# gyhandy/Neural-Sim-NeRF

Measured on AMD Instinct MI355X. Metric: Mray-samples/sec at 400x400, 64+128 samples, 8x256 MLP, higher is better.
Workload: dtype f16x2

## Files before the change

### neural_sim_nerf_amd/csrc/nsr_kernels.hip

```cpp
#include <hip/hip_runtime.h>
#include <stdint.h>
#include "nsr_device.h"

#if !defined(NSR_UNIT_F32) && !defined(NSR_UNIT_H2) && !defined(NSR_UNIT_B3) && !defined(NSR_UNIT_X16)
#define NSR_UNIT_F32 1
#define NSR_UNIT_H2 1
#define NSR_UNIT_B3 1
#define NSR_UNIT_X16 1
#endif
#ifndef NSR_UNIT_F32
#define NSR_UNIT_F32 0
#endif
#ifndef NSR_UNIT_H2
#define NSR_UNIT_H2 0
#endif
#ifndef NSR_UNIT_B3
#define NSR_UNIT_B3 0
#endif
#ifndef NSR_UNIT_X16
#define NSR_UNIT_X16 0
#endif
#define NSR_CAT_(a, b) a##b
#define NSR_CAT(a, b) NSR_CAT_(a, b)

// ... 88 lines not shown
#pragma unroll
  for (int c = 0; c < 4; ++c) A0[c] = *(const f32x4*)(p + c * 1024);
}

template <int U>
__device__ __forceinline__ void ring_load_quarter(const Ring& rg, f32x4 (&A)[4], int lane) {
  const char* p = rg.smem + rg.cslot * kSlabBytes + U * kStepBytes + lane * 16;
#pragma unroll
  for (int c = 0; c < 4; ++c) A[c] = *(const f32x4*)(p + c * 1024);
}

template <int NS = kRingSlots>
__device__ __forceinline__ void ring_advance(Ring& rg, f32x4 (&A)[4], int lane) {
  asm volatile("s_waitcnt vmcnt(%0) lgkmcnt(0)" ::"n"(4 * (NS - 2)) : "memory");
#ifndef NSR_EXP_NOBARRIER
  __builtin_amdgcn_s_barrier();
#endif
  rg.cslot = (rg.cslot + 1 == NS) ? 0 : rg.cslot + 1;
  const char* p = rg.smem + rg.cslot * kSlabBytes + lane * 16;
#pragma unroll
  for (int c = 0; c < 4; ++c) A[c] = *(const f32x4*)(p + c * 1024);
}

#define NSR_MFMA(a, b, c) __builtin_amdgcn_mfma_f32_32x32x2f32((a), (b), (c), 0, 0, 0)
__device__ __forceinline__ f32x16 mfma_op(float a, float b, f32x16 c) { return __builtin_amdgcn_mfma_f32_32x32x2f32(a, b, c, 0, 0, 0); }
__device__ __forceinline__ f32x4 mfma_op(float a, float b, f32x4 c) { return __builtin_amdgcn_mfma_f32_16x16x4f32(a, b, c, 0, 0, 0); }

template <int NMO, int KK0, int KK1, bool ZERO = false, int NACC, typename BOp, typename AccT>
__device__ __forceinline__ void consume(const f32x4 (&A)[4], int step, BOp bop, AccT (&acc)[NACC]) {
#pragma unroll
  for (int kk = KK0; kk < KK1; ++kk)
#pragma unroll
    for (int c = 0; c < 4; ++c) {
      const int n = 4 * step + c, tq = n / NMO, mo = n % NMO;
      if (ZERO && tq == 0 && kk == 0) acc[mo] = mfma_op(A[c][kk], bop(4 * tq + kk), AccT{0});
      else acc[mo] = mfma_op(A[c][kk], bop(4 * tq + kk), acc[mo]);
    }
}

#define NSR_PIN() __builtin_amdgcn_sched_barrier(0)
#define NSR_SGB(mask, n) __builtin_amdgcn_sched_group_barrier((mask), (n), 0)
#define NSR_MASK_VALU 0x002
#define NSR_MASK_SALU 0x004
#define NSR_MASK_MFMA 0x008
#define NSR_MASK_VMEM 0x010
#define NSR_MASK_DSRD 0x100
template <int N_MFMA>
__device__ __forceinline__ void step_pattern() {
#pragma unroll
  for (int i = 0; i < N_MFMA; ++i) {
    NSR_SGB(NSR_MASK_MFMA, 1);
    NSR_SGB(NSR_MASK_DSRD, 1);
    NSR_SGB(NSR_MASK_VALU, 2);
  }
}
template <int N_MFMA>
__device__ __forceinline__ void step_pattern_dma() {
#pragma unroll
  for (int i = 0; i < N_MFMA; ++i) {
    NSR_SGB(NSR_MASK_MFMA, 1);
    NSR_SGB(NSR_MASK_DSRD, 1);
    NSR_SGB(NSR_MASK_VMEM, 1);
    NSR_SGB(NSR_MASK_SALU, 3);
    NSR_SGB(NSR_MASK_VALU, 2);
  }
}

template <int NMO, int NTQ, int NS = kRingSlots, bool ZERO = false, int NACC, typename BOp, typename AccT>
__device__ __forceinline__ void seg(Ring& rg, f32x4 (&A0)[4], f32x4 (&A1)[4], BOp bop, AccT (&acc)[NACC],
                                    int lane) {
  static_assert((NMO * NTQ) % 16 == 0, "a segment is a whole number of slabs");
#pragma unroll
  for (int s = 0; s < NMO * NTQ / 4; s += 4) {
    NSR_PIN(); ring_load_quarter<1>(rg, A1, lane); consume<NMO, 0, 4, ZERO>(A0, s, bop, acc);     step_pattern<16>();
    NSR_PIN(); ring_load_quarter<2>(rg, A0, lane); consume<NMO, 0, 4, ZERO>(A1, s + 1, bop, acc); step_pattern<16>();
    NSR_PIN(); ring_load_quarter<3>(rg, A1, lane); consume<NMO, 0, 4, ZERO>(A0, s + 2, bop, acc); step_pattern<16>();
    NSR_PIN(); consume<NMO, 0, 1, ZERO>(A1, s + 3, bop, acc);
    NSR_PIN(); ring_advance<NS>(rg, A0, lane);
    ring_issue<NS>(rg); consume<NMO, 1, 4, ZERO>(A1, s + 3, bop, acc); step_pattern_dma<12>();
    NSR_PIN();
  }
}

template <int NG>
struct BRegs16 {
  const f32x16 (&v)[NG];
  __device__ __forceinline__ float operator()(int t) const { return v[t >> 4][t & 15]; }
};
template <int N>
struct BArr {
  const float (&v)[N];
  __device__ __forceinline__ float operator()(int t) const { return v[t]; }
};
struct BViews {
  const f32x16 (&v)[8];
  const float (&ed)[16];
  __device__ __forceinline__ float operator()(int t) const { return t < 128 ? v[(t & 127) >> 4][t & 15] : ed[t & 15]; }
};

__device__ __forceinline__ int aux_half(int lane) { return opaque_v((lane >> 5) * 4); }

template <int NMO>
__device__ __forceinline__ void load_bias(const float* bias, int h4 , f32x16 (&acc)[NMO]) {
#pragma unroll
  for (int mo = 0; mo < NMO; ++mo)
#pragma unroll
    for (int rq = 0; rq < 4; ++rq) {
      f32x4 v = *(const f32x4*)(bias + (mo * 4 + rq) * 8 + h4);
      acc[mo][rq * 4 + 0] = v[0];
      acc[mo][rq * 4 + 1] = v[1];
      acc[mo][rq * 4 + 2] = v[2];
      acc[mo][rq * 4 + 3] = v[3];
    }
}

#include "nsr_b3.inc"
#include "nsr_h2.inc"

constexpr int kMlpF32 = 0;
constexpr int kMlpB3 = 1;
constexpr int kMlpH2 = 2;

template <int NMO>
__device__ __forceinline__ uint4 relu_mask(const f32x16 (&acc)[NMO]) {
  unsigned w[4] = {0u, 0u, 0u, 0u};
#pragma unroll
  for (int mo = 0; mo < NMO; ++mo)
#pragma unroll
    for (int r = 0; r < 16; ++r) {
      const int on = max(__float_as_int(acc[mo][r]), 0) - 1;
      w[mo >> 1] = __builtin_amdgcn_alignbit(w[mo >> 1], (unsigned)on, 31);
    }
  return make_uint4(w[0], w[1], w[2], w[3]);
}

__device__ __forceinline__ float enc_trig(float a, int k) {
  const double kMagic = 6755399441055744.0;
  const double t = (double)a * 0.63661977236758134308;
  const double tm = t + kMagic;
  const int n = __double2loint(tm) + k;
  const double f = t - (tm - kMagic);
  const float r = (float)(f * 1.57079632679489661923);
  const float z = r * r;
  float ps = __builtin_fmaf(-1.9515295891e-4f, z, 8.3321608736e-3f);
  ps = __builtin_fmaf(ps, z, -1.6666654611e-1f);
  ps = __builtin_fmaf(ps * z, r, r);
  float pc = __builtin_fmaf(2.443315711809948e-5f, z, -1.388731625493765e-3f);
  pc = __builtin_fmaf(pc, z, 4.166664568298827e-2f);
  pc = __builtin_fmaf(pc * z, z, __builtin_fmaf(-0.5f, z, 1.0f));
  const float v = (n & 1) ? pc : ps;
  return __uint_as_float(__float_as_uint(v) ^ ((unsigned)(n & 2) << 30));
}

__device__ __forceinline__ float enc_domain(float x, int nfreq) {
  return __builtin_fabsf(x) < ldexpf(1.0f, 25 - nfreq) ? x : __builtin_nanf("");
}

__device__ __forceinline__ float enc_poison(float px, float py, float pz, float vx, float vy, float vz) {
  const float a = (enc_domain(px, kMultires) * 0.0f + enc_domain(py, kMultires) * 0.0f) + enc_domain(pz, kMultires) * 0.0f;
  const float b = (enc_domain(vx, kMultiresViews) * 0.0f + enc_domain(vy, kMultiresViews) * 0.0f) +
                  enc_domain(vz, kMultiresViews) * 0.0f;
  return __builtin_fabsf(a + b);
}

template <bool CAPTURE, int MODE = kMlpF32>
__device__ __forceinline__ void mlp_pass(Ring& rg, const float* aux, f32x4 (&A0)[4], f32x4 (&A1)[4], int lane,
                                         float px, float py, float pz, float vx, float vy, float vz,
                                         float (&raw)[4], uint4* mask_dst = nullptr , int mask_tid = 0,
                                         long long* tp = nullptr ) {
#ifdef NSR_PHASE_TIMING
  long long tpl = clock64();
#define NSR_TP(i) do { if (tp) { const long long t_ = clock64(); tp[i] += t_ - tpl; tpl = t_; } } while (0)
#else
#define NSR_TP(i) do { } while (0)
#endif
  const int h = lane >> 5;
  const int h4 = aux_half(lane);
  const float poison = enc_poison(px, py, pz, vx, vy, vz);
  float e[32];
  float ed[16];
  {
    const float p[3] = {px, py, pz};
    const float v[3] = {vx, vy, vz};
#pragma unroll
    for (int L = 0; L < kMultires; ++L)
#pragma unroll
      for (int ax = 0; ax < 3; ++ax) e[3 * L + ax] = enc_trig(enc_domain(p[ax], kMultires) * (float)(1 << L), h);
#pragma unroll
    for (int L = 0; L < kMultiresViews; ++L)
#pragma unroll
      for (int ax = 0; ax < 3; ++ax) ed[3 * L + ax] = enc_trig(enc_domain(v[ax], kMultiresViews) * (float)(1 << L), h);
    e[30] = h ? pz : px;
    e[31] = h ? 0.0f : py;
    ed[12] = h ? vz : vx;
    ed[13] = h ? 0.0f : vy;
    ed[14] = 0.0f;
    ed[15] = 0.0f;
  }

  f32x16 acc[8];
  f32x16 in[8];
  auto enc_src = [&](int kb, int i) { return e[(8 * kb + i) & 31]; };
  auto in_src = [&](int kb, int i) { return in[(kb >> 1) & 7][8 * (kb & 1) + i]; };
  constexpr bool B3 = MODE == kMlpB3;
  constexpr bool H2M = MODE == kMlpH2;
  float amax = 0.0f;
  const float* h2s = aux + kAuxH2Scale;
#if NSR_H2_SCHED == 3 && !defined(NSR_EXP_H2_NOFRAG) && !defined(NSR_EXP_H2_HALFBARRIER) && !defined(NSR_EXP_H2_NOSPLIT)
  constexpr bool TAIL = H2M && !CAPTURE;
#else
  constexpr bool TAIL = false;
#endif
  static_assert(kAuxBiasV == kAuxBias + 9 * 256, "the views layer's bias follows feature_linear's: 'bias of layer L + 1' for L = 8");
  NSR_TP(0);
  load_bias<8>(aux + kAuxBias, h4, acc);
  NSR_TP(2);
  if constexpr (B3) gemm_b3<8, 2>(rg, A0, A1, enc_src, acc, lane);
  else if constexpr (TAIL)
    gemm_h2_tail<4>(rg, A0, A1, enc_src, H2Scale{{h2s[0], 0.0f}, 4}, acc, lane, amax, H2Tail{acc, in, 0, h2_lds_base(aux + kAuxBias + 256, h4)});
  else if constexpr (H2M) gemm_h2<8, 4>(rg, A0, A1, enc_src, H2Scale{{h2s[0], 0.0f}, 4}, acc, lane, amax);
  else seg<8, 8>(rg, A0, A1, BArr<32>{e}, acc, lane);
  NSR_TP(1);
  if (CAPTURE) mask_dst[mask_tid] = relu_mask<8>(acc);
  if constexpr (!TAIL) {
#pragma unroll
    for (int mo = 0; mo < 8; ++mo) in[mo] = relu16(acc[mo]);
  }

  float alpha_part = 0.0f;
#pragma unroll 1
  for (int L = 1; L <= 8; ++L) {
    if constexpr (!TAIL) load_bias<8>(aux + kAuxBias + L * 256, h4, acc);
    NSR_TP(2);
    if (L == 5) {
      if constexpr (B3) gemm_b3<8, 2>(rg, A0, A1, enc_src, acc, lane);
      else if constexpr (H2M) gemm_h2<8, 4>(rg, A0, A1, enc_src, H2Scale{{h2s[9], 0.0f}, 4}, acc, lane, amax);
      else seg<8, 8>(rg, A0, A1, BArr<32>{e}, acc, lane);
      NSR_TP(1);
    }
    if (L == 8) {
      const float* wa = aux + kAuxWAlpha;
#pragma unroll
      for (int tq = 0; tq < 32; ++tq) {
        f32x4 w = *(const f32x4*)(wa + tq * 8 + h4);
#pragma unroll
        for (int kk = 0; kk < 4; ++kk)
          alpha_part = __builtin_fmaf(w[kk], in[(4 * tq + kk) >> 4][(4 * tq + kk) & 15], alpha_part);
      }
    }
    if constexpr (B3) gemm_b3<8, 8>(rg, A0, A1, in_src, acc, lane);
    else if constexpr (TAIL)
      gemm_h2_tail<16>(rg, A0, A1, in_src, H2Scale{{h2s[L], 0.0f}, 16}, acc, lane, amax,
                       H2Tail{acc, in, (L == 8) ? (int)0x80000000 : 0, h2_lds_base(aux + kAuxBias + (L + 1) * 256, h4)});
    else if constexpr (H2M) gemm_h2<8, 16>(rg, A0, A1, in_src, H2Scale{{h2s[L], 0.0f}, 16}, acc, lane, amax);
    else seg<8, 32>(rg, A0, A1, BRegs16<8>{in}, acc, lane);
    NSR_TP(1);
    if (CAPTURE && L < 8) mask_dst[L * 256 + mask_tid] = relu_mask<8>(acc);
    if constexpr (!TAIL) {
      const int thr = (L == 8) ? (int)0x80000000 : 0;
#pragma unroll
      for (int mo = 0; mo < 8; ++mo) in[mo] = clamp_bits16(acc[mo], thr);
    }
  }

  f32x16 av[4];
  if constexpr (TAIL) {
#pragma unroll
    for (int mo = 0; mo < 4; ++mo) av[mo] = acc[mo];
  } else {
    load_bias<4>(aux + kAuxBiasV, h4, av);
  }
  NSR_TP(2);
  if constexpr (B3) {
    auto v_src = [&](int kb, int i) {
      return kb < 16 ? in[(kb >> 1) & 7][8 * (kb & 1) + i] : (kb < 18 ? ed[(8 * (kb - 16) + i) & 15] : 0.0f);
    };
    gemm_b3<4, 5>(rg, A0, A1, v_src, av, lane);
  } else if constexpr (H2M) {
    auto v_src = [&](int kb, int i) { return kb < 16 ? in[(kb >> 1) & 7][8 * (kb & 1) + i] : ed[(8 * (kb - 16) + i) & 15]; };
    gemm_h2<4, 18>(rg, A0, A1, v_src, H2Scale{{h2s[10], h2s[11]}, 16}, av, lane, amax);
  } else {
    seg<4, 36>(rg, A0, A1, BViews{in, ed}, av, lane);
  }
  NSR_TP(1);
  if (CAPTURE) mask_dst[8 * 256 + mask_tid] = relu_mask<4>(av);

  float part[4] = {0.0f, 0.0f, 0.0f, alpha_part};
  if constexpr (H2M) {
    const float ov = amax > kH2Max ? __builtin_nanf("") : 0.0f;
    part[0] = part[1] = part[2] = ov;
    part[3] = alpha_part + ov;
  }
#pragma unroll
  for (int c = 0; c < 3; ++c) {
    const float* wr = aux + kAuxWRgb + c * 128;
#pragma unroll
    for (int mo = 0; mo < 4; ++mo)
#pragma unroll
      for (int rq = 0; rq < 4; ++rq) {
        f32x4 w = *(const f32x4*)(wr + (mo * 4 + rq) * 8 + h4);
#pragma unroll
        for (int ri = 0; ri < 4; ++ri)
          part[c] = __builtin_fmaf(w[ri], fmaxf(av[mo][rq * 4 + ri], 0.0f), part[c]);
      }
  }
#pragma unroll
  for (int c = 0; c < 4; ++c) {
    float other = __shfl_xor(part[c], 32);
    float lo_half = h ? other : part[c];
    float hi_half = h ? part[c] : other;
    raw[c] = ((lo_half + hi_half) + aux[(c < 3) ? (kAuxBRgb + c) : kAuxBAlpha]) + poison;
  }
  NSR_TP(3);
#undef NSR_TP
}

template <int NSS, int NFS>
struct ItemStateT {
  static constexpr int kNS = NSS, kNF = NFS;
  float tcoarse[NSS];
  float ufine[128];
  float ray[2][16];
  float zc[2][NSS];
  float rawc[2][NSS][4];
  float w0[2][NSS];
  float cdf[2][NSS];
  float zs[2][128];
  float zf[2][NFS];
  float rawf[2][NFS][4];
  float alpha[2][NFS];
  float wf[2][NFS];
  float tf[2][NFS];
  float om[2][NFS];
  float bwd_scratch[2][NFS][2];
  float psum[2][NFS / 32][12];
  float gnorm[2];
  float res[2][8];
};
typedef ItemStateT<64, 192> ItemState;
typedef ItemStateT<128, 256> ItemStateBig;
static_assert(sizeof(ItemState) == 23048, "the YCB-V layout is part of the shipped kernels' LDS budget");
template <int NS> struct ItemStateFor { typedef ItemState type; };
template <> struct ItemStateFor<128> { typedef ItemStateBig type; };

__device__ __forceinline__ float sigmoidf_(float x) { return 1.0f / (1.0f + expf(-x)); }

template <int S, int R = 2, int STRIDE = S, typename ST>
__device__ __forceinline__ void composite(ST& st, const float* z, float* raw, float* wout, float* tout, int tid,
                                          const float* noise = nullptr ,
                                          long long row0 = 0, int valid = R) {
  static_assert(S % 8 == 0, "scan is unrolled by 8");
  for (int idx = tid; idx < R * S; idx += 256) {
    const int r = idx / S, i = idx - r * S;
    const float* zr = z + r * STRIDE;
    float dist = (i < S - 1) ? (zr[i + 1] - zr[i]) : 1e10f;
    dist = dist * st.ray[r][11];
    float* q = raw + (r * STRIDE + i) * 4;
    if (noise) q[3] = q[3] + noise[(row0 + (r < valid ? r : 0)) * S + i];
    const float sigma = fmaxf(q[3], 0.0f);
    const float a = 1.0f - expf(-sigma * dist);
    st.alpha[r][i] = a;
    st.om[r][i] = (1.0f - a) + 1e-10f;
    q[0] = sigmoidf_(q[0]);
    q[1] = sigmoidf_(q[1]);
    q[2] = sigmoidf_(q[2]);
  }
  __syncthreads();
  if ((tid & 63) == 0 && tid < 64 * R) {
    const int r = tid >> 6;
    double T = 1.0;
#pragma unroll 1
    for (int i0 = 0; i0 < S; i0 += 8) {
      double f[8];
#pragma unroll
      for (int k = 0; k < 8; ++k) f[k] = (double)st.om[r][i0 + k];
#pragma unroll
      for (int k = 0; k < 8; ++k) {
        tout[r * STRIDE + i0 + k] = (float)T;
        T = T * f[k];
      }
    }
  }
  __syncthreads();
  if (tid < 64 * R) {
    const int r = tid >> 6, l = tid & 63;
    const float* zr = z + r * STRIDE;
    const float* q = raw + r * STRIDE * 4;
    float cr = 0.f, cg = 0.f, cb = 0.f, depth = 0.f, acc = 0.f;
#pragma unroll
    for (int i = l; i < S; i += 64) {
      const float w = st.alpha[r][i] * tout[r * STRIDE + i];
      wout[r * STRIDE + i] = w;
      cr = cr + w * q[i * 4 + 0];
      cg = cg + w * q[i * 4 + 1];
      cb = cb + w * q[i * 4 + 2];
      depth = depth + w * zr[i];
      acc = acc + w;
    }
#pragma unroll
    for (int m = 32; m >= 1; m >>= 1) {
      cr += __shfl_xor(cr, m); cg += __shfl_xor(cg, m); cb += __shfl_xor(cb, m);
      depth += __shfl_xor(depth, m); acc += __shfl_xor(acc, m);
    }
    if (l == 0) {
      const float qd = depth / acc;
      float disp;
      if (qd != qd) disp = qd;
      else disp = 1.0f / fmaxf(1e-10f, qd);
      if (st.ray[r][12] != 0.0f) {
        const float bg = 1.0f - acc;
        cr = cr + bg; cg = cg + bg; cb = cb + bg;
      }
      st.res[r][0] = cr; st.res[r][1] = cg; st.res[r][2] = cb;
      st.res[r][3] = disp; st.res[r][4] = acc; st.res[r][5] = depth;
    }
  }
  __syncthreads();
}
// ... 253 lines not shown
      const float upper = i < NS - 1 ? 0.5f * (zr[i + 1] + zr[i]) : zr[NS - 1];
      zn = lower + (upper - lower) * t_rand[(row0 + (r < valid ? r : 0)) * NS + i];
    }
    __syncthreads();
    if (tid < 2 * NS) st.zc[r][i] = zn;
    __syncthreads();
  }
}

__device__ __forceinline__ void gen_ray(const float* __restrict__ c2w, float fx, float fy, float cx, float cy,
                                        int row, int col, float (&o)[3], float (&d)[3]) {
  const float dx = ((float)col - cx) / fx;
  const float dy = -(((float)row - cy) / fy);
  const float dz = -1.0f;
#pragma unroll
  for (int a = 0; a < 3; ++a) {
    d[a] = ((dx * c2w[a * 4 + 0]) + (dy * c2w[a * 4 + 1])) + (dz * c2w[a * 4 + 2]);
    o[a] = c2w[a * 4 + 3];
  }
}

struct RenderArgs {
  const float* nets;
  long long net_stride;
  const float* aux[2];
  const float* tcoarse;
  const float* ufine;
  const float* rays_o;
  const float* rays_d;
  const float* c2w;
  float fx, fy, cx, cy;
  int H, W;
  long long n_rays;
  float near_, far_;
  int fine;
  int camera;
  int white_bkgd;
  int lindisp;
  float *rgb, *disp, *acc, *rgb0, *disp0, *acc0, *z_std;
  float *dbg_w0, *dbg_zs, *dbg_zf, *dbg_raw0, *dbg_raw;
  long long* dbg_inds;
  float* zf_scratch;
  int chunk;
  unsigned* sched_flags;
  unsigned* status;
  int super_lg;
  int spin_max;
  unsigned epoch;
  unsigned* epoch_counter;
  unsigned long long* work_counter;
  const float* viewdirs;
  const float* t_rand;
  const float* u_rays;
  const float* noise0;
  const float* noise1;
  const float* near_rays;
  const float* far_rays;
  unsigned long long* ovf_items;
  unsigned* ovf_stat;
  unsigned ovf_cap;
  const unsigned long long* item_list;
  const unsigned* item_count;
  unsigned item_cap;
};

__device__ __forceinline__ void load_aux(char* smem, const RenderArgs& a, int tid) {
  float* dst = (float*)(smem + kLdsAux);
  for (int i = tid; i < kAuxFloats; i += 256) {
    dst[i] = a.aux[0][i];
    dst[kAuxFloats + i] = a.aux[1][i];
  }
}

#if NSR_UNIT_F32
__global__ void k_set_args(const RenderArgs a, RenderArgs* dst) {
  *dst = a;
  *a.work_counter = 0ull;
  if (a.ovf_stat) a.ovf_stat[0] = 0u;
  if (a.epoch_counter) dst->epoch = *a.epoch_counter = *a.epoch_counter % 4094u + 1u;
}
#endif

constexpr long long kItemMask = (1ll << 62) - 1;
__device__ __forceinline__ long long queue_next_item(const RenderArgs& q) {
  const unsigned long long v = atomicAdd(q.work_counter, 1ull);
  if (q.item_list) {
    unsigned n = *q.item_count;
    n = n < q.item_cap ? n : q.item_cap;
    return v < (unsigned long long)n ? (long long)q.item_list[v] : -1ll;
  }
  return v < (unsigned long long)((q.n_rays + 1) >> 1) ? (long long)(v | (3ull << 62)) : -1ll;
}
__device__ __forceinline__ long long queue_item_of(const RenderArgs& q, unsigned long long v) {
  if (q.item_list) {
    unsigned n = *q.item_count;
    n = n < q.item_cap ? n : q.item_cap;
    return v < (unsigned long long)n ? (long long)q.item_list[v] : -1ll;
  }
  return v < (unsigned long long)((q.n_rays + 1) >> 1) ? (long long)(v | (3ull << 62)) : -1ll;
}
__device__ __forceinline__ long long queue_items(const RenderArgs& q) {
  if (q.item_list) { const unsigned n = *q.item_count; return (long long)(n < q.item_cap ? n : q.item_cap); }
  return (q.n_rays + 1) >> 1;
}
__device__ __forceinline__ void range_mark(int* ovf, float chk, int lane) {
#ifndef NSR_EXP_NO_RANGE
  if (chk != chk && lane < 32) atomicAdd(ovf, 1);
#endif
}
__device__ __forceinline__ unsigned range_report(const RenderArgs& a, int* ovf, long long item, int valid) {
#ifdef NSR_EXP_NO_RANGE
  return 0u;
#endif
  const int p0 = ovf[0], p1 = valid == 2 ? ovf[1] : 0;
  if ((p0 | p1) != 0 && a.ovf_stat) {
    const unsigned long long mask = (p0 ? 1ull : 0ull) | (p1 ? 2ull : 0ull);
    const unsigned n = atomicAdd(a.ovf_stat, 1u);
    atomicAdd(a.ovf_stat + 1, (unsigned)(p0 + p1));
    if (n < a.ovf_cap) {
      a.ovf_items[n] = (unsigned long long)item | (mask << 62);
      atomicAdd(a.ovf_stat + 2, (unsigned)((p0 != 0) + (p1 != 0)));
    } else {
      atomicAdd(a.ovf_stat + 3, 1u);
      return (unsigned)mask;
    }
  }
  return 0u;
}
__device__ __forceinline__ void range_poison(const RenderArgs& a, long long ray0, unsigned mask) {
  const float qn = __builtin_nanf("");
  for (int r = 0; r < 2; ++r) {
    if (!((mask >> r) & 1u)) continue;
    const long long rr = ray0 + r;
    float* const v3[2] = {a.rgb, a.rgb0};
    float* const v1[5] = {a.disp, a.acc, a.disp0, a.acc0, a.z_std};
    for (int k = 0; k < 2; ++k) if (v3[k]) { v3[k][rr * 3] = qn; v3[k][rr * 3 + 1] = qn; v3[k][rr * 3 + 2] = qn; }
    for (int k = 0; k < 5; ++k) if (v1[k]) v1[k][rr] = qn;
  }
}

__device__ __forceinline__ void wave_lds_sync() {
  __builtin_amdgcn_fence(__ATOMIC_RELEASE, "wavefront");
  __builtin_amdgcn_wave_barrier();
  __builtin_amdgcn_fence(__ATOMIC_ACQUIRE, "wavefront");
}
__device__ __forceinline__ void lds_barrier() { asm volatile("s_waitcnt lgkmcnt(0)\n\ts_barrier" ::: "memory"); }

template <typename ST>
struct FwdItemExtra {
  float om[2][ST::kNS];
  float tf[2][ST::kNS];
  float zf[2][ST::kNF];
  float ray[2][16];
  float res[2][8];
  long long pend;
  long long next;
};

template <int S>
__device__ __forceinline__ void composite_wave(const float* ry, const float* zr, float* q, float* wr, float* tr, float* omr,
                                               int lane, const float* noise ,
                                               float (&res)[6]) {
  static_assert(S % 8 == 0, "scan is unrolled by 8");
  constexpr int K = (S + 63) / 64;
  float al[K];
#pragma unroll
  for (int k = 0; k < K; ++k) {
    const int i = lane + 64 * k;
    al[k] = 0.0f;
    if (i < S) {
      float dist = (i < S - 1) ? (zr[i + 1] - zr[i]) : 1e10f;
      dist = dist * ry[11];
      if (noise) q[i * 4 + 3] = q[i * 4 + 3] + noise[i];
      const float sigma = fmaxf(q[i * 4 + 3], 0.0f);
      const float a = 1.0f - expf(-sigma * dist);
      al[k] = a;
      omr[i] = (1.0f - a) + 1e-10f;
      q[i * 4 + 0] = sigmoidf_(q[i * 4 + 0]);
      q[i * 4 + 1] = sigmoidf_(q[i * 4 + 1]);
      q[i * 4 + 2] = sigmoidf_(q[i * 4 + 2]);
    }
  }
  wave_lds_sync();
  if (lane == 0) {
    double T = 1.0;
#pragma unroll 1
    for (int i0 = 0; i0 < S; i0 += 8) {
      double f[8];
#pragma unroll
      for (int k = 0; k < 8; ++k) f[k] = (double)omr[i0 + k];
#pragma unroll
      for (int k = 0; k < 8; ++k) {
        tr[i0 + k] = (float)T;
        T = T * f[k];
      }
    }
  }
  wave_lds_sync();
  float cr = 0.f, cg = 0.f, cb = 0.f, depth = 0.f, acc = 0.f;
#pragma unroll
  for (int k = 0; k < K; ++k) {
    const int i = lane + 64 * k;
    if (i < S) {
      const float w = al[k] * tr[i];
      wr[i] = w;
      cr = cr + w * q[i * 4 + 0];
      cg = cg + w * q[i * 4 + 1];
      cb = cb + w * q[i * 4 + 2];
      depth = depth + w * zr[i];
      acc = acc + w;
    }
  }
#pragma unroll
  for (int m = 32; m >= 1; m >>= 1) {
    cr += __shfl_xor(cr, m); cg += __shfl_xor(cg, m); cb += __shfl_xor(cb, m);
    depth += __shfl_xor(depth, m); acc += __shfl_xor(acc, m);
  }
  const float qd = depth / acc;
  float disp;
  if (qd != qd) disp = qd;
  else disp = 1.0f / fmaxf(1e-10f, qd);
  if (ry[12] != 0.0f) {
    const float bg = 1.0f - acc;
    cr = cr + bg; cg = cg + bg; cb = cb + bg;
  }
  res[0] = cr; res[1] = cg; res[2] = cb; res[3] = disp; res[4] = acc; res[5] = depth;
  wave_lds_sync();
}

template <int NI, int NS>
__device__ __forceinline__ void sample_pdf_wave(const float* w, const float* zc, float* x, float* pdf, float* cdf, float* zs,
                                                const float* u ,
                                                int64_t* inds_out , int lane) {
  constexpr int NW = NS - 2, NC = NS - 1;
  constexpr int NVEC = NW / 8, SILP = NVEC / 4;
  constexpr int KW = (NW + 63) / 64;
  float xv[KW];
#pragma unroll
  for (int k = 0; k < KW; ++k) {
    const int i = lane + 64 * k;
    xv[k] = 0.0f;
    if (i < NW) { xv[k] = w[i] + 1e-5f; x[i] = xv[k]; }
  }
  wave_lds_sync();
  const int j = lane & 7;
  float lj;
  if constexpr (NS == 64) {
    const float p0 = ((x[j] + x[32 + j]) + x[40 + j]) + x[48 + j];
    lj = ((p0 + x[8 + j]) + x[16 + j]) + x[24 + j];
  } else {
    float ps[4] = {0.0f, 0.0f, 0.0f, 0.0f};
#pragma unroll
    for (int i = 0; i < SILP; ++i)
#pragma unroll
      for (int k = 0; k < 4; ++k) ps[k] = ps[k] + x[(i * 4 + k) * 8 + j];
#pragma unroll
    for (int v = SILP * 4; v < NVEC; ++v) ps[0] = ps[0] + x[v * 8 + j];
    lj = ((ps[0] + ps[1]) + ps[2]) + ps[3];
  }
  float total = 0.0f;
#pragma unroll
  for (int i = NVEC * 8; i < NW; ++i) total = total + x[i];
#pragma unroll
  for (int jj = 0; jj < 8; ++jj) total = total + __shfl(lj, jj);
#pragma unroll
  for (int k = 0; k < KW; ++k) {
    const int i = lane + 64 * k;
    if (i < NW) pdf[i] = xv[k] / total;
  }
  wave_lds_sync();
  if (lane == 0) {
    double run = 0.0;
    cdf[0] = 0.0f;
#pragma unroll 1
    for (int i0 = 0; i0 < NVEC * 8; i0 += 8) {
      double f[8];
#pragma unroll
      for (int k = 0; k < 8; ++k) f[k] = (double)pdf[i0 + k];
#pragma unroll
      for (int k = 0; k < 8; ++k) { run = run + f[k]; cdf[i0 + k + 1] = (float)run; }
    }
#pragma unroll
    for (int i = NVEC * 8; i < NW; ++i) { run = run + (double)pdf[i]; cdf[i + 1] = (float)run; }
  }
  wave_lds_sync();
#pragma unroll
  for (int kk = 0; kk < (NI + 63) / 64; ++kk) {
    const int k = lane + 64 * kk;
    if (k < NI) {
      const float uu = u[k];
      int lo = 0, hi = NC;
      while (lo < hi) {
        const int mid = (lo + hi) >> 1;
        if (cdf[NSR_IDX(mid, NC)] <= uu) lo = mid + 1; else hi = mid;
      }
      const int ind = lo;
      const int below = NSR_IDX(max(ind - 1, 0), NC);
      const int above = NSR_IDX(min(ind, NC - 1), NC);
      const float c0 = cdf[below], c1 = cdf[above];
      const float b0 = 0.5f * (zc[below + 1] + zc[below]), b1 = 0.5f * (zc[above + 1] + zc[above]);
      float denom = c1 - c0;
      if (denom < 1e-5f) denom = 1.0f;
      const float t = (uu - c0) / denom;
      zs[NSR_IDX(k, 128)] = b0 + t * (b1 - b0);
      if (inds_out) inds_out[k] = (int64_t)ind;
    }
  }
  wave_lds_sync();
}

template <int NI, int NS>
__device__ __forceinline__ void merge_wave(const float* zc, const float* zs, float* zf, int lane) {
  constexpr int NF = NS + NI;
  constexpr bool kPow2 = (NI & (NI - 1)) == 0 && (NS & (NS - 1)) == 0;
  constexpr int K = (NF + 63) / 64;
  int bad = 0;
#pragma unroll
  for (int kk = 0; kk < K; ++kk) {
    const int k = lane + 64 * kk;
    if (k < NS - 1) bad |= !(zc[k] <= zc[k + 1]);
    else if (k >= NS && k < NF - 1) bad |= !(zs[k - NS] <= zs[k - NS + 1]);
  }
  const bool any_bad = __builtin_amdgcn_ballot_w64(bad != 0) != 0;
  if (!any_bad) {
#pragma unroll
    for (int kk = 0; kk < K; ++kk) {
      const int k = lane + 64 * kk;
      if (k < NS) {
        const float x = zc[k];
        int lb = 0;
        if constexpr (kPow2) {
#pragma unroll
          for (int sft = NI / 2; sft > 0; sft >>= 1) lb += (zs[lb + sft - 1] < x) ? sft : 0;
          lb += (zs[lb] < x) ? 1 : 0;
        } else {
          int hi = NI;
          while (lb < hi) { const int mid = (lb + hi) >> 1; if (zs[NSR_IDX(mid, NI)] < x) lb = mid + 1; else hi = mid; }
        }
        zf[NSR_IDX(k + lb, NF)] = x;
      } else if (k < NF) {
        const float x = zs[k - NS];
        int ub = 0;
        if constexpr (kPow2) {
#pragma unroll
          for (int sft = NS / 2; sft > 0; sft >>= 1) ub += (zc[ub + sft - 1] <= x) ? sft : 0;
          ub += (zc[ub] <= x) ? 1 : 0;
        } else {
          int hi = NS;
          while (ub < hi) { const int mid = (ub + hi) >> 1; if (zc[NSR_IDX(mid, NS)] <= x) ub = mid + 1; else hi = mid; }
        }
        zf[NSR_IDX((k - NS) + ub, NF)] = x;
      }
    }
  } else {
#pragma unroll 1
    for (int kk = 0; kk < K; ++kk) {
      const int k = lane + 64 * kk;
      if (k < NF) {
        const float x = (k < NS) ? zc[k] : zs[k - NS];
        int rank = 0;
        for (int jx = 0; jx < NS; ++jx) {
          const float y = zc[jx];
          rank += (y < x) || (y == x && jx < k);
        }
        for (int jx = 0; jx < NI; ++jx) {
          const float y = zs[jx];
          rank += (y < x) || (y == x && (jx + NS) < k);
        }
        zf[NSR_IDX(rank, NF)] = x;
      }
    }
  }
  wave_lds_sync();
}

#ifdef NSR_PHASE_TIMING
#define NSR_T(i) do { if (threadIdx.x == 0) { const long long t_ = clock64(); tacc[i] += t_ - tlast; tlast = t_; } } while (0)
#else
#define NSR_T(i) do { } while (0)
#endif

template <int MODE, int NI = 128, int NS = 64>
__device__ __forceinline__ void render32_body(const RenderArgs* __restrict__ ap, char* smem) {
  constexpr bool B3 = MODE == kMlpB3;
  constexpr int NF = NS + NI;
  constexpr int NP = (2 * NF + 127) / 128;
  constexpr int NPC = (2 * NS + 127) / 128;
  constexpr int LNS = NS == 32 ? 5 : (NS == 64 ? 6 : 7);
  typedef typename ItemStateFor<NS>::type ST;
  static_assert((NS == 32 || NS == 64 || NS == 128) && NF % 32 == 0 && NS <= ST::kNS && NF <= ST::kNF,
                "a wave's points belong to one ray; the item state holds kNS coarse / kNF fine samples per ray");
  const RenderArgs& a_setup = *ap;
#ifdef NSR_PHASE_TIMING
  long long tacc[8] = {0, 0, 0, 0, 0, 0, 0, 0};
  long long tpass[4] = {0, 0, 0, 0};
  long long tlast = clock64();
#define NSR_TPASS tpass
#else
#define NSR_TPASS nullptr
#endif
  const int tid0 = threadIdx.x;
  const int lane = tid0 & 63;
  const int wave = __builtin_amdgcn_readfirstlane(tid0 >> 6);
  const int j = lane & 31;
  ST& st = *(ST*)(smem + kLdsState);

  const long long n_rays = a_setup.n_rays;
  if ((long long)blockIdx.x >= queue_items(a_setup)) return;
  const int fine = a_setup.fine;
  typedef FwdItemExtra<ST> XT;
  static_assert(offsetof(ST, res) - offsetof(ST, bwd_scratch) >= sizeof(XT) && offsetof(ST, bwd_scratch) % 8 == 0 &&
                offsetof(XT, pend) % 8 == 0, "the forward scratch lives in the item state's backward scratch");
  XT& xs = *(XT*)&st.bwd_scratch[0][0][0];

  Ring rg;
  ring_init(rg, smem, a_setup.nets, a_setup.net_stride, fine ? NPC + NP : NPC, wave, lane);
  rg.pn0 = NPC; rg.pn1 = NPC + NP;

  f32x4 A0[4], A1[4];
  if constexpr (B3) ring_start<kRingSlots, kStreamSlabsB3, kStreamSlabsB3Bwd>(rg, A0, lane);
  else if constexpr (MODE == kMlpH2) ring_start<kRingSlots, kStreamSlabs, kStreamSlabs, kH2RingLag>(rg, A0, lane);
  else ring_start(rg, A0, lane);

  load_aux(smem, a_setup, tid0);
  if (tid0 < NS) st.tcoarse[tid0] = a_setup.tcoarse[tid0];
  if (tid0 < NI) st.ufine[tid0] = a_setup.ufine[tid0];
  if (tid0 == 0) xs.pend = -1ll;
  __syncthreads();
  const float* aux_c = (const float*)(smem + kLdsAux);

  long long* item_slot = (long long*)&st.ray[0][14];
  auto next_item = [&]() -> long long {
    if (opaque_v(tid0) == 0) *item_slot = queue_next_item(*opaque_s(ap));
    lds_barrier();
    const long long v = uniform64(*item_slot);
    lds_barrier();
    return v;
  };

  auto fine_wave = [&](long long pk, int pp, int r) {
    const RenderArgs& a = *opaque_s(ap);
    const long long ray0 = (pk & kItemMask) * 2;
    const int valid = (ray0 + 1 < n_rays) ? 2 : 1;
    const int wmask = (int)((unsigned long long)pk >> 62) & (valid == 2 ? 3 : 1);
    const float* ry = pp ? xs.ray[r] : st.ray[r];
    const float* zr = pp ? xs.zf[r] : st.zf[r];
    float* q = &st.rawf[r][0][0];
    if (a.dbg_raw && ((wmask >> r) & 1)) {
      for (int idx = lane; idx < NF * 4; idx += 64) a.dbg_raw[(ray0 + r) * (NF * 4) + idx] = q[idx];
      wave_lds_sync();
    }
    float res[6];
    composite_wave<NF>(ry, zr, q, st.wf[r], st.tf[r], st.om[r], lane,
                       a.noise1 ? a.noise1 + (ray0 + (r < valid ? r : 0)) * NF : nullptr, res);
    if (lane == 0) {
#pragma unroll
      for (int c = 0; c < 6; ++c) st.res[r][c] = res[c];
    }
  };
  auto fine_out = [&](long long pk, int pp) {
    const RenderArgs& a = *opaque_s(ap);
    const int tid = opaque_v(tid0);
    const long long item = pk & kItemMask;
    const long long ray0 = item * 2;
    const int valid = (ray0 + 1 < n_rays) ? 2 : 1;
    const int wmask = (int)((unsigned long long)pk >> 62) & (valid == 2 ? 3 : 1);
    if (tid < 16 && ((wmask >> (tid >> 3)) & 1)) {
      const int r = tid >> 3, c = tid & 7;
      const long long rr = ray0 + r;
      const float v = st.res[r][c];
      if (c < 3) { if (a.rgb) a.rgb[rr * 3 + c] = v; }
      else if (c == 3) { if (a.disp) a.disp[rr] = v; }
      else if (c == 4) { if (a.acc) a.acc[rr] = v; }
    }
    if (MODE == kMlpH2 && tid == 0) {
      int* povf = (int*)(pp ? &xs.ray[1][14] : &st.ray[1][14]);
      if (const unsigned m = range_report(a, povf, item, valid)) range_poison(a, ray0, m);
    }
  };

  long long packed = next_item();
  int pass = 0;
  int par = 0;
#pragma unroll 1
  while (packed != -1ll) {
    const long long item = packed & kItemMask;
    const long long ray0 = item * 2;
    const int valid = (ray0 + 1 < n_rays) ? 2 : 1;
    const int wmask = (int)((unsigned long long)packed >> 62) & (valid == 2 ? 3 : 1);
    auto wr = [&](int r) { return ((wmask >> r) & 1) != 0; };
    float (*const ray)[16] = par ? xs.ray : st.ray;
    float* const zf = par ? &xs.zf[0][0] : &st.zf[0][0];
    int* const ovf = (int*)&ray[1][14];
    if (pass == 0) {
      const RenderArgs& a = *opaque_s(ap);
      const int tid = opaque_v(tid0);
      const float near_ = a.near_, far_ = a.far_;
      if (tid < 2) {
        const long long rr = ray0 + (tid < valid ? tid : 0);
        float o[3], d[3];
        if (a.camera) {
          const long long hw = (long long)a.H * a.W;
          const long long v = rr / hw;
          const int pix = (int)(rr - v * hw);
          gen_ray(a.c2w + v * 12, a.fx, a.fy, a.cx, a.cy, pix / a.W, pix % a.W, o, d);
        } else {
#pragma unroll
          for (int c = 0; c < 3; ++c) { o[c] = a.rays_o[rr * 3 + c]; d[c] = a.rays_d[rr * 3 + c]; }
        }
        const float nrm = sqrtf(((d[0] * d[0]) + (d[1] * d[1])) + (d[2] * d[2]));
        const float* vd = a.camera ? nullptr : a.viewdirs;
#pragma unroll
        for (int c = 0; c < 3; ++c) {
          ray[tid][c] = o[c]; ray[tid][3 + c] = d[c];
          ray[tid][6 + c] = vd ? vd[rr * 3 + c] : d[c] / nrm;
        }
        ray[tid][9] = a.near_rays ? a.near_rays[rr] : near_;
        ray[tid][10] = a.near_rays ? a.far_rays[rr] : far_;
        ray[tid][11] = nrm;
        ray[tid][12] = a.white_bkgd ? 1.0f : 0.0f;
      }
      if (MODE == kMlpH2 && (tid == 64 || tid == 65)) ovf[tid - 64] = 0;
      if (tid < 2 * NS) {
        const int r = tid >> LNS, i = tid & (NS - 1);
        const float t = st.tcoarse[i];
        const long long rb = ray0 + (r < valid ? r : 0);
        st.zc[r][i] = coarse_z(a.near_rays ? a.near_rays[rb] : near_, a.near_rays ? a.far_rays[rb] : far_, t, a.lindisp);
      }
      lds_barrier();
      if (a.t_rand) perturb_coarse_z<NS>(st, a.t_rand, ray0, valid, tid);
      NSR_T(0);
    }

    {
      int r, i;
      const float* zsrc;
      float* dst;
      bool real = true;
      if ((NPC == 1) ? (pass == 0) : (pass < NPC)) {
        if constexpr (NS == 64) {
          r = wave >> 1; i = 32 * (wave & 1) + j;
        } else {
          int q0 = 128 * pass + 32 * wave;
          if (2 * NS % 128 != 0 && q0 >= 2 * NS) { q0 = 2 * NS - 32; real = false; }
          r = q0 >> LNS; i = (q0 & (NS - 1)) + j;
        }
        zsrc = &st.zc[r][i]; dst = st.rawc[r][i];
      } else {
        int q0 = 128 * (pass - NPC) + 32 * wave;
        if (2 * NF % 128 != 0 && q0 >= 2 * NF) { q0 = 2 * NF - 32; real = false; }
        r = q0 / NF; i = q0 - r * NF + j;
        zsrc = &zf[r * ST::kNF + i]; dst = st.rawf[r][i];
      }
      const float z = *zsrc;
      const float* ry = ray[r];
      float raw[4];
      mlp_pass<false, MODE>(rg, aux_c + (((NPC == 1) ? (pass == 0) : (pass < NPC)) ? 0 : kAuxFloats), A0, A1, lane, ry[0] + ry[3] * z, ry[1] + ry[4] * z,
               ry[2] + ry[5] * z, ry[6], ry[7], ry[8], raw, nullptr, 0, NSR_TPASS);
      if (lane < 32 && real) *(f32x4*)dst = f32x4{raw[0], raw[1], raw[2], raw[3]};
      if constexpr (MODE == kMlpH2) { if (real) range_mark(ovf + r, (raw[0] + raw[1]) + (raw[2] + raw[3]), lane); }
    }
    NSR_T(1);

    const RenderArgs& a = *opaque_s(ap);
    const int tid = opaque_v(tid0);
    if (NPC > 1 && pass < NPC - 1) {
      ++pass;
    } else if ((NPC == 1) ? (pass == 0) : (pass < NPC)) {
      lds_barrier();
      const long long pend = fine ? uniform64(xs.pend) : -1ll;
      const bool puller = fine && tid == 192;
      unsigned long long ticket = 0ull;
      if (puller) ticket = atomicAdd(a.work_counter, 1ull);
      if (wave < 2) {
        const int r = wave;
        float* q = &st.rawc[r][0][0];
        if (a.dbg_raw0 && wr(r)) {
          for (int idx = lane; idx < NS * 4; idx += 64) a.dbg_raw0[(ray0 + r) * (NS * 4) + idx] = q[idx];
          wave_lds_sync();
        }
        float res[6];
        composite_wave<NS>(ray[r], st.zc[r], q, st.w0[r], xs.tf[r], xs.om[r], lane,
                           a.noise0 ? a.noise0 + (ray0 + (r < valid ? r : 0)) * NS : nullptr, res);
        if (lane == 0) {
#pragma unroll
          for (int c = 0; c < 6; ++c) xs.res[r][c] = res[c];
        }
        if (a.dbg_w0 && wr(r))
          for (int idx = lane; idx < NS; idx += 64) a.dbg_w0[(ray0 + r) * NS + idx] = st.w0[r][idx];
        NSR_T(2);
        if (fine) {
#ifdef NSR_PHASE_TIMING
          int64_t* inds = nullptr;
#else
          int64_t* inds = (int64_t*)a.dbg_inds;
#endif
          sample_pdf_wave<NI, NS>(&st.w0[r][1], st.zc[r], xs.tf[r], xs.om[r], st.cdf[r], st.zs[r],
                                  a.u_rays ? a.u_rays + (ray0 + (r < valid ? r : 0)) * 128 : st.ufine,
                                  (inds && wr(r)) ? inds + (ray0 + r) * NI : nullptr, lane);
          NSR_T(3);
          const float sd = zstd_wave<NI>(st, r, lane);
          if (lane == 0 && wr(r) && a.z_std) a.z_std[ray0 + r] = sd;
          if (a.dbg_zs && wr(r))
            for (int k = lane; k < NI; k += 64) a.dbg_zs[(ray0 + r) * NI + k] = st.zs[r][k];
          NSR_T(4);
          merge_wave<NI, NS>(st.zc[r], st.zs[r], zf + r * ST::kNF, lane);
          if (a.dbg_zf && wr(r))
            for (int k = lane; k < NF; k += 64) a.dbg_zf[(ray0 + r) * NF + k] = zf[r * ST::kNF + k];
          NSR_T(5);
        }
      } else if (pend != -1ll) {
#ifdef NSR_PHASE_TIMING
        const long long t0_ = clock64();
#endif
        fine_wave(pend, par ^ 1, wave - 2);
#ifdef NSR_PHASE_TIMING
        if (threadIdx.x == 128) tacc[7] += clock64() - t0_;
#endif
      }
      if (puller) xs.next = queue_item_of(a, ticket);
      lds_barrier();
      if (pend != -1ll) fine_out(pend, par ^ 1);
      if (tid < 16 && wr(tid >> 3)) {
        const int r = tid >> 3, c = tid & 7;
        const long long rr = ray0 + r;
        const float v = xs.res[r][c];
        float* rgb_dst = fine ? a.rgb0 : a.rgb;
        float* disp_dst = fine ? a.disp0 : a.disp;
        float* acc_dst = fine ? a.acc0 : a.acc;
        if (c < 3) { if (rgb_dst) rgb_dst[rr * 3 + c] = v; }
        else if (c == 3) { if (disp_dst) disp_dst[rr] = v; }
        else if (c == 4) { if (acc_dst) acc_dst[rr] = v; }
      }
      NSR_T(6);
      if (!fine) {
        if (MODE == kMlpH2 && tid == 0) { if (const unsigned m = range_report(a, ovf, item, valid)) range_poison(a, ray0, m); }
        if constexpr (NPC > 1) pass = 0;
        packed = next_item(); continue;
      }
      pass = NPC;
    } else if (pass < NPC + NP - 1) {
      ++pass;
    } else {
      if (tid == 0) xs.pend = packed;
      pass = 0;
      par ^= 1;
      packed = uniform64(xs.next);
    }
  }
  if (fine) {
    lds_barrier();
    const long long pend = uniform64(xs.pend);
    if (pend != -1ll) {
      if (wave < 2) fine_wave(pend, par ^ 1, wave);
      lds_barrier();
      fine_out(pend, par ^ 1);
    }
    NSR_T(6);
  }
  asm volatile("s_waitcnt vmcnt(0)" ::: "memory");
#ifdef NSR_PHASE_TIMING
  if (tid0 == 128 && a_setup.dbg_raw == nullptr && a_setup.dbg_inds) a_setup.dbg_inds[blockIdx.x * 8 + 7] = tacc[7];
  if (tid0 == 0 && a_setup.dbg_raw == nullptr && a_setup.dbg_inds)
    for (int i = 0; i < 7; ++i) a_setup.dbg_inds[blockIdx.x * 8 + i] = tacc[i];
  if (tid0 == 0 && a_setup.dbg_raw == nullptr && a_setup.dbg_inds)
    for (int i = 0; i < 4; ++i) a_setup.dbg_inds[(long long)gridDim.x * 8 + blockIdx.x * 4 + i] = tpass[i];
#endif
#undef NSR_TPASS
}

#define NSR_RENDER_KERNEL_1(NAME, ...)                                                               \
  __global__ void __launch_bounds__(256, 1) NAME(const RenderArgs* __restrict__ ap) {                \
    extern __shared__ __attribute__((aligned(16))) char smem[];                                      \
    render32_body<__VA_ARGS__>(ap, smem);                                                            \
  }
#define NSR_RENDER_KERNEL_0(NAME, ...) __global__ void __launch_bounds__(256, 1) NAME(const RenderArgs* __restrict__ ap);
#define NSR_RENDER_KERNEL(UNIT, NAME, ...) NSR_CAT(NSR_RENDER_KERNEL_, UNIT)(NAME, __VA_ARGS__)
NSR_RENDER_KERNEL(NSR_UNIT_F32, k_render, kMlpF32)
NSR_RENDER_KERNEL(NSR_UNIT_B3, k_render_b3, kMlpB3)
NSR_RENDER_KERNEL(NSR_UNIT_H2, k_render_h2, kMlpH2)
NSR_RENDER_KERNEL(NSR_UNIT_H2, k_render_h2_n64, kMlpH2, 64)
NSR_RENDER_KERNEL(NSR_UNIT_H2, k_render_h2_n32, kMlpH2, 32)
NSR_RENDER_KERNEL(NSR_UNIT_B3, k_render_b3_n64, kMlpB3, 64)
NSR_RENDER_KERNEL(NSR_UNIT_B3, k_render_b3_n32, kMlpB3, 32)
NSR_RENDER_KERNEL(NSR_UNIT_H2, k_render_h2_n96, kMlpH2, 96, 64)
NSR_RENDER_KERNEL(NSR_UNIT_B3, k_render_b3_n96, kMlpB3, 96, 64)
NSR_RENDER_KERNEL(NSR_UNIT_H2, k_render_h2_c32_n64, kMlpH2, 64, 32)
NSR_RENDER_KERNEL(NSR_UNIT_B3, k_render_b3_c32_n64, kMlpB3, 64, 32)
NSR_RENDER_KERNEL(NSR_UNIT_H2, k_render_h2_c128_n128, kMlpH2, 128, 128)
NSR_RENDER_KERNEL(NSR_UNIT_B3, k_render_b3_c128_n128, kMlpB3, 128, 128)
#undef NSR_RENDER_KERNEL
#undef NSR_RENDER_KERNEL_0
#undef NSR_RENDER_KERNEL_1

__device__ __forceinline__ f32x16 apply_mask(f32x16 x, unsigned word, int shift) {
  f32x16 r;
#pragma unroll
  for (int i = 0; i < 16; ++i)
    r[i] = ((word >> (31 - (shift + i))) & 1u) ? 0.0f : x[i];
  return r;
}

template <int NFREQ>
__device__ __forceinline__ void embed_bwd(const float (&x)[3], const float* G , int h,
                                          float (&out)[3]) {
  out[0] = h ? 0.0f : G[3 * NFREQ];
  out[1] = h ? 0.0f : G[3 * NFREQ + 1];
  out[2] = h ? G[3 * NFREQ] : 0.0f;
#pragma unroll
  for (int L = 0; L < NFREQ; ++L)
#pragma unroll
// ... 1797 lines not shown
```

Measured before the change: 279.0.

## Share sin/cos range reduction and precompute per-ray view-direction encodings in LDS

The positional encoding now computes sine and cosine from one range reduction per angle, with each lane half handling half the frequencies and a permlane32 swap exchanging results. This halves the per-sample trig work. View-direction encodings are constant along a ray, so they are computed once per ray by a few threads at setup, stored in LDS scratch and read back as float4s in the forward pass. This adds LDS space, a cross-lane swap and extra setup work in exchange for fewer per-sample trig evaluations.

```diff
diff --git a/neural_sim_nerf_amd/csrc/nsr_kernels.hip b/neural_sim_nerf_amd/csrc/nsr_kernels.hip
--- a/neural_sim_nerf_amd/csrc/nsr_kernels.hip
+++ b/neural_sim_nerf_amd/csrc/nsr_kernels.hip
@@ -264,6 +264,26 @@
   return __uint_as_float(__float_as_uint(v) ^ ((unsigned)(n & 2) << 30));
 }
 
+__device__ __forceinline__ void enc_trig2(float a, float& s, float& c) {
+  const double kMagic = 6755399441055744.0;
+  const double t = (double)a * 0.63661977236758134308;
+  const double tm = t + kMagic;
+  const int n = __double2loint(tm);
+  const double f = t - (tm - kMagic);
+  const float r = (float)(f * 1.57079632679489661923);
+  const float z = r * r;
+  float ps = __builtin_fmaf(-1.9515295891e-4f, z, 8.3321608736e-3f);
+  ps = __builtin_fmaf(ps, z, -1.6666654611e-1f);
+  ps = __builtin_fmaf(ps * z, r, r);
+  float pc = __builtin_fmaf(2.443315711809948e-5f, z, -1.388731625493765e-3f);
+  pc = __builtin_fmaf(pc, z, 4.166664568298827e-2f);
+  pc = __builtin_fmaf(pc * z, z, __builtin_fmaf(-0.5f, z, 1.0f));
+  const float vs = (n & 1) ? pc : ps;
+  const float vc = ((n + 1) & 1) ? pc : ps;
+  s = __uint_as_float(__float_as_uint(vs) ^ ((unsigned)(n & 2) << 30));
+  c = __uint_as_float(__float_as_uint(vc) ^ ((unsigned)((n + 1) & 2) << 30));
+}
+
 __device__ __forceinline__ float enc_domain(float x, int nfreq) {
   return __builtin_fabsf(x) < ldexpf(1.0f, 25 - nfreq) ? x : __builtin_nanf("");
 }
@@ -275,11 +295,13 @@
   return __builtin_fabsf(a + b);
 }
 
-template <bool CAPTURE, int MODE = kMlpF32>
+template <bool CAPTURE, int MODE = kMlpF32, bool RAYENC = false>
 __device__ __forceinline__ void mlp_pass(Ring& rg, const float* aux, f32x4 (&A0)[4], f32x4 (&A1)[4], int lane,
                                          float px, float py, float pz, float vx, float vy, float vz,
                                          float (&raw)[4], uint4* mask_dst = nullptr , int mask_tid = 0,
-                                         long long* tp = nullptr ) {
+                                         long long* tp = nullptr ,
+                                         const float* edr = nullptr ) {
+  static_assert(!(RAYENC && CAPTURE), "the input-gradient kernels keep the per-lane encodings");
 #ifdef NSR_PHASE_TIMING
   long long tpl = clock64();
 #define NSR_TP(i) do { if (tp) { const long long t_ = clock64(); tp[i] += t_ - tpl; tpl = t_; } } while (0)
@@ -294,14 +316,27 @@
   {
     const float p[3] = {px, py, pz};
     const float v[3] = {vx, vy, vz};
-#pragma unroll
-    for (int L = 0; L < kMultires; ++L)
-#pragma unroll
-      for (int ax = 0; ax < 3; ++ax) e[3 * L + ax] = enc_trig(enc_domain(p[ax], kMultires) * (float)(1 << L), h);
-#pragma unroll
-    for (int L = 0; L < kMultiresViews; ++L)
-#pragma unroll
-      for (int ax = 0; ax < 3; ++ax) ed[3 * L + ax] = enc_trig(enc_domain(v[ax], kMultiresViews) * (float)(1 << L), h);
+    if constexpr (RAYENC) {
+      static_assert(kMultires == 10 && kMultiresViews == 4, "15 + 15 position angles, 12 direction angles in three float4s");
+      const int up = h4 * (5 << 21);
+#pragma unroll
+      for (int i = 0; i < 15; ++i) {
+        float s, c;
+        enc_trig2(enc_domain(p[i % 3], kMultires) * __int_as_float(((127 + i / 3) << 23) + up), s, c);
+        const auto sw = __builtin_amdgcn_permlane32_swap(__float_as_uint(s), __float_as_uint(c), false, false);
+        e[i] = __uint_as_float(sw[0]);
+        e[15 + i] = __uint_as_float(sw[1]);
+      }
+    } else {
+#pragma unroll
+      for (int L = 0; L < kMultires; ++L)
+#pragma unroll
+        for (int ax = 0; ax < 3; ++ax) e[3 * L + ax] = enc_trig(enc_domain(p[ax], kMultires) * (float)(1 << L), h);
+#pragma unroll
+      for (int L = 0; L < kMultiresViews; ++L)
+#pragma unroll
+        for (int ax = 0; ax < 3; ++ax) ed[3 * L + ax] = enc_trig(enc_domain(v[ax], kMultiresViews) * (float)(1 << L), h);
+    }
     e[30] = h ? pz : px;
     e[31] = h ? 0.0f : py;
     ed[12] = h ? vz : vx;
@@ -376,6 +411,15 @@
   }
 
   f32x16 av[4];
+  if constexpr (RAYENC) {
+    const f32x4* ev = (const f32x4*)(edr + 4 * h4);
+#pragma unroll
+    for (int q = 0; q < 3; ++q) {
+      const f32x4 w = ev[q];
+#pragma unroll
+      for (int k = 0; k < 4; ++k) ed[4 * q + k] = w[k];
+    }
+  }
   if constexpr (TAIL) {
 #pragma unroll
     for (int mo = 0; mo < 4; ++mo) av[mo] = acc[mo];
@@ -935,6 +979,7 @@
   float tf[2][ST::kNS];
   float zf[2][ST::kNF];
   float ray[2][16];
+  float ed[2][2][32];
   float res[2][8];
   long long pend;
   long long next;
@@ -1194,6 +1239,8 @@
   typedef FwdItemExtra<ST> XT;
   static_assert(offsetof(ST, res) - offsetof(ST, bwd_scratch) >= sizeof(XT) && offsetof(ST, bwd_scratch) % 8 == 0 &&
                 offsetof(XT, pend) % 8 == 0, "the forward scratch lives in the item state's backward scratch");
+  constexpr bool RAYENC = true;
+  static_assert((kLdsState + offsetof(ST, bwd_scratch) + offsetof(XT, ed)) % 16 == 0, "mlp_pass reads a ray's direction encodings as float4s");
   XT& xs = *(XT*)&st.bwd_scratch[0][0][0];
 
   Ring rg;
@@ -1279,8 +1326,11 @@
       const RenderArgs& a = *opaque_s(ap);
       const int tid = opaque_v(tid0);
       const float near_ = a.near_, far_ = a.far_;
-      if (tid < 2) {
-        const long long rr = ray0 + (tid < valid ? tid : 0);
+      const bool encl = RAYENC && tid >= 64 && tid < 128 && (tid & 15) < 12;
+      float vc = 0.0f;
+      if (tid < 2 || encl) {
+        const int rs = encl ? ((tid >> 5) & 1) : tid;
+        const long long rr = ray0 + (rs < valid ? rs : 0);
         float o[3], d[3];
         if (a.camera) {
           const long long hw = (long long)a.H * a.W;
@@ -1293,15 +1343,26 @@
         }
         const float nrm = sqrtf(((d[0] * d[0]) + (d[1] * d[1])) + (d[2] * d[2]));
         const float* vd = a.camera ? nullptr : a.viewdirs;
-#pragma unroll
-        for (int c = 0; c < 3; ++c) {
-          ray[tid][c] = o[c]; ray[tid][3 + c] = d[c];
-          ray[tid][6 + c] = vd ? vd[rr * 3 + c] : d[c] / nrm;
-        }
-        ray[tid][9] = a.near_rays ? a.near_rays[rr] : near_;
-        ray[tid][10] = a.near_rays ? a.far_rays[rr] : far_;
-        ray[tid][11] = nrm;
-        ray[tid][12] = a.white_bkgd ? 1.0f : 0.0f;
+        float vdir[3];
+#pragma unroll
+        for (int c = 0; c < 3; ++c) vdir[c] = vd ? vd[rr * 3 + c] : d[c] / nrm;
+        if (!encl) {
+#pragma unroll
+          for (int c = 0; c < 3; ++c) {
+            ray[tid][c] = o[c]; ray[tid][3 + c] = d[c];
+            ray[tid][6 + c] = vdir[c];
+          }
+          ray[tid][9] = a.near_rays ? a.near_rays[rr] : near_;
+          ray[tid][10] = a.near_rays ? a.far_rays[rr] : far_;
+          ray[tid][11] = nrm;
+          ray[tid][12] = a.white_bkgd ? 1.0f : 0.0f;
+        }
+        const int ax = (tid & 15) % 3;
+        vc = ax == 0 ? vdir[0] : (ax == 1 ? vdir[1] : vdir[2]);
+      }
+      if (encl) {
+        const int r = (tid >> 5) & 1, hh = (tid >> 4) & 1, t = tid & 15;
+        xs.ed[par][r][16 * hh + t] = enc_trig(enc_domain(vc, kMultiresViews) * (float)(1 << (t / 3)), hh);
       }
       if (MODE == kMlpH2 && (tid == 64 || tid == 65)) ovf[tid - 64] = 0;
       if (tid < 2 * NS) {
@@ -1338,8 +1399,8 @@
       const float z = *zsrc;
       const float* ry = ray[r];
       float raw[4];
-      mlp_pass<false, MODE>(rg, aux_c + (((NPC == 1) ? (pass == 0) : (pass < NPC)) ? 0 : kAuxFloats), A0, A1, lane, ry[0] + ry[3] * z, ry[1] + ry[4] * z,
-               ry[2] + ry[5] * z, ry[6], ry[7], ry[8], raw, nullptr, 0, NSR_TPASS);
+      mlp_pass<false, MODE, RAYENC>(rg, aux_c + (((NPC == 1) ? (pass == 0) : (pass < NPC)) ? 0 : kAuxFloats), A0, A1, lane, ry[0] + ry[3] * z, ry[1] + ry[4] * z,
+               ry[2] + ry[5] * z, ry[6], ry[7], ry[8], raw, nullptr, 0, NSR_TPASS, xs.ed[par][r]);
       if (lane < 32 && real) *(f32x4*)dst = f32x4{raw[0], raw[1], raw[2], raw[3]};
       if constexpr (MODE == kMlpH2) { if (real) range_mark(ovf + r, (raw[0] + raw[1]) + (raw[2] + raw[3]), lane); }
     }
```

After: 280.9, median of 6. No clear change (+0.7%).
